# mozack/vdjer

Hardware: AMD Instinct MI355X
Metric: M paired-reads/sec (k-mer build + contig score), IgH 50bp PE (higher is better)
Workload: dtype u8/u64 (2-bit packed bases, integer counts)

## Files before the change

### vdjer_amd/csrc/vdjx_kmer.hip

```cpp
#include "vdjx_common.h"
#include "vdjx_scan.h"
#include "vdjx_part.h"

#include <algorithm>
#include <numeric>
#include <type_traits>
#include <string.h>
#include <stdlib.h>

#define HIST_THREADS 512
#define HIST_BLOCKS 512u
#define LOCAL_SLOTS 2048u
#define K3_SUB_TUPLES g_sub_tuples
__device__ u32 g_sub_tuples = 262144u;
#define NONE32 0xFFFFFFFFu
#define INST_MASK 0x7FFFFFFFu

struct RecView {
	u64 bhi, blo, nm, lq;
};

__device__ inline RecView load_rec(const u64* __restrict__ bases, const u64* __restrict__ nmask,
                                   const u64* __restrict__ lowq, size_t r) {
	RecView v;
// ... 1124 lines not shown
	if (r0 == NONE32) return;
	if ((need & NEED_SEQ) && r != r0 && lane == 0) {
		const u64* a = (const u64*) me;
		const u64* b = (const u64*) (replies + (size_t) r0 * REPLY_BYTES);
		u64 d = 0;
#pragma unroll
		for (int w = 2; w < 10; w++) d |= a[w] ^ b[w];
		if (d) p_fl[pid] = 1;
	}
	if ((need & NEED_Q) && (int) lane < k) {
		const uint8_t* first = me + REPLY_Q0 + (r == r0 ? 2 * REPLY_KQ : REPLY_KQ);
		atomicAdd(&p_S[(size_t) pid * 64 + lane], (u32) me[REPLY_Q0 + lane] + (u32) first[lane]);
		if (np) {
			const uint8_t* first_r = me + REPLY_RQ0 + (r == p_r0[np + pid] ? 2 * REPLY_KQ : REPLY_KQ);
			atomicAdd(&p_S[((size_t) np + pid) * 64 + lane], (u32) me[REPLY_RQ0 + lane] + (u32) first_r[lane]);
		}
	}
}

template <bool SYM>
__global__ void k_resolve_keep(PendOut po, u32 np, const u32* __restrict__ p_fl, const u32* __restrict__ p_S, int k, u32 mf, u32 mqq, u32 tlow,
                               SurvOutG so) {
	const u32 p = blockIdx.x * blockDim.x + threadIdx.x;
	const bool in = p < np;
	const u32 need = in ? po.need[p] : 0u;
	bool keep = in && ((need & NEED_SEQ) ? p_fl[p] != 0 : true);
	const u32 cg = in ? po.cg[p] : 0u;
	const u32 cgc = cg > CNT_CAP ? CNT_CAP : cg;
	keep = keep && cgc >= mf;
	bool keep_r = keep;
	if (keep && cg < tlow) {
		for (int j = 0; j < k; j++) if (p_S[(size_t) p * 64 + j] < mqq) { keep = false; break; }
		if (SYM) for (int j = 0; j < k; j++) if (p_S[((size_t) np + p) * 64 + j] < mqq) { keep_r = false; break; }
	}
	if (!SYM) {
		const u32 pos = vdjx_wave_inc(so.n, keep);
		if (keep && pos < so.cap) {
			so.lo[pos] = po.lo[p]; so.hi[pos] = po.hi[p];
			so.gcnt[pos] = cgc; so.gfirst[pos] = po.mg[p];
		}
		return;
	}
	const bool any = keep || keep_r;
	const u32 pos = vdjx_wave_inc(so.n, any, 2u);
	if (any && pos + 1 < so.cap) {
		so.lo[pos] = po.lo[p]; so.hi[pos] = po.hi[p];
		so.gcnt[pos] = cgc | (keep ? 0u : GC_SHADOW); so.gfirst[pos] = po.mg[p];
		u64 rh, rlo;
		vdjx_kmer_rc(po.hi[p], po.lo[p], k, rh, rlo);
		so.lo[pos + 1] = rlo; so.hi[pos + 1] = rh;
		so.gcnt[pos + 1] = cgc | (keep_r ? 0u : GC_SHADOW); so.gfirst[pos + 1] = po.mgr[p];
	}
}

__global__ void k_first_to_scan(u64* __restrict__ a, size_t na, u64* __restrict__ b, size_t nb, const u32* __restrict__ scan, int ob) {
	const size_t i = (size_t) blockIdx.x * blockDim.x + threadIdx.x;
	if (i >= na + nb) return;
	u64* p = i < na ? a + i : b + (i - na);
	const u64 v = *p;
	if (v != NONE64) *p = ((u64) scan[v >> ob] << ob) | (v & ((1ull << ob) - 1ull));
}

__global__ void k_node_flags(const u64* __restrict__ s_lo, const u64* __restrict__ s_hi, u32 n, int k,
                             const u32* __restrict__ vbits, const u32* __restrict__ jbits,
                             uint8_t* __restrict__ has_v, uint8_t* __restrict__ has_j) {
	u32 i = blockIdx.x * blockDim.x + threadIdx.x;
	if (i >= n) return;
	if (k <= 16) { has_v[i] = 1; has_j[i] = 1; return; }
	u128 key = ((u128) s_hi[i] << 64) | s_lo[i];
	u32 code = (u32) (key >> (2 * (k - 16)));
	has_v[i] = code ? (vbits[code >> 5] >> (code & 31)) & 1u : 0;
	has_j[i] = code ? (jbits[code >> 5] >> (code & 31)) & 1u : 0;
}


#define IT_INST_BITS 35
#define IT_INST_MASK ((1ull << IT_INST_BITS) - 1ull)
#define IT_SURV_SHIFT 38
#define IT_HOLE 0xFFFFFFFFFFFFFFFFull
#define WALK_THREADS 256

#define SLOT_HI_BITS 36
#define SLOT_HI_MASK ((1ull << SLOT_HI_BITS) - 1ull)
struct SurvTable { const ulonglong2* slots; u32 mask; const ulonglong2* skey; const u32* bloom; u32 bloom_mask; };

struct ItemFmt {
	u32 pmask;
	u32 len_shift;
	u32 maxlen;
	u32 mul, inv;
	u32 bmask;
	u32 ns;
};
__device__ inline u32 it_surv(const ItemFmt& f, u64 x) { return (u32) (x >> IT_SURV_SHIFT) & f.pmask; }
__device__ inline u32 it_len(const ItemFmt& f, u64 x) { return f.maxlen > 1 ? (u32) (x >> f.len_shift) + 1u : 1u; }
__device__ inline u32 it_scat(const ItemFmt& f, u32 p) { return ((((p >> 4) * f.mul) & f.bmask) << 4) | (p & 15u); }

__global__ void k_surv_table2(const u64* __restrict__ s_lo, const u64* __restrict__ s_hi, u32 n, ulonglong2* __restrict__ slots, u32 mask,
                              ulonglong2* __restrict__ skey, u32* __restrict__ bloom, u32 bloom_mask) {
	const u32 i = blockIdx.x * blockDim.x + threadIdx.x;
	if (i >= n) return;
	const u64 lo = s_lo[i], hi = s_hi[i];
	skey[i] = make_ulonglong2(lo, hi);
	const u64 h = vdjx_mix(lo, hi);
	{
		const u32 bit = (u32) (h >> 40) & bloom_mask;
		atomicOr(&bloom[bit >> 5], 1u << (bit & 31));
	}
	u32 slot = (u32) (h >> 20) & mask;
	const unsigned long long entry = hi | ((unsigned long long) (i + 1) << SLOT_HI_BITS);
	while (atomicCAS((unsigned long long*) &slots[slot].y, 0ull, entry) != 0ull) slot = (slot + 1) & mask;
	slots[slot].x = lo;
}

__device__ inline int surv_lookup2f(const SurvTable& t, u64 lo, u64 hi);

__device__ inline int surv_lookup2(const SurvTable& t, u64 lo, u64 hi) {
	u32 slot = (u32) (vdjx_mix(lo, hi) >> 20) & t.mask;
	for (;;) {
		const ulonglong2 v = t.slots[slot];
		if (!v.y) return -1;
		if (v.x == lo && (v.y & SLOT_HI_MASK) == hi) return (int) (v.y >> SLOT_HI_BITS) - 1;
		slot = (slot + 1) & t.mask;
	}
}

__device__ inline int surv_lookup2f(const SurvTable& t, u64 lo, u64 hi) {
	const u64 h = vdjx_mix(lo, hi);
	const u32 bit = (u32) (h >> 40) & t.bloom_mask;
	if (!((t.bloom[bit >> 5] >> (bit & 31)) & 1u)) return -1;
	return surv_lookup2(t, lo, hi);
}

__global__ void k_succ_links2(SurvTable t, u32 n, int k, const u32* __restrict__ gcnt, u32* __restrict__ succ, unsigned long long* __restrict__ pred,
                              u32* __restrict__ bestsucc) {
	const u32 u = blockIdx.x * blockDim.x + threadIdx.x;
	if (u >= n) return;
	const ulonglong2 kk = t.skey[u];
	const u128 base = (((u128) kk.y << 64) | kk.x) << 2;
	const u128 km = k < 64 ? (((u128) 1) << (2 * k)) - 1 : ~(u128) 0;
	const int sh = 2 * (k - 1);
	const u32 fb = (u32) (sh < 64 ? kk.x >> sh : kk.y >> (sh - 64)) & 3u;
	const unsigned long long mine = ((unsigned long long) (gcnt[u] & GC_MASK) << 32) | ((unsigned long long) (fb ^ 1u) << 30) | (unsigned long long) u;
	u32 best = NONE32, best_g = 0;
	for (u32 b = 0; b < 4; b++) {
		const u128 key = (base | (u128) b) & km;
		const int s = surv_lookup2(t, (u64) key, (u64) (key >> 64));
		succ[u * 4 + b] = s >= 0 ? (u32) s : NONE32;
		if (s >= 0 && (u32) s != u) {
			const u32 g = gcnt[s] & GC_MASK;
			if (best == NONE32 || g >= best_g) { best = (u32) s; best_g = g; }
			atomicMax(&pred[s], mine);
		}
	}
	bestsucc[u] = best;
}

#define CHAIN_JUMPS 31
__global__ void k_chain_init(const unsigned long long* __restrict__ pred, const u32* __restrict__ bestsucc, u32 n, u64* __restrict__ pd) {
	const u32 v = blockIdx.x * blockDim.x + threadIdx.x;
	if (v >= n) return;
	const unsigned long long x = pred[v];
	const u32 u = (u32) x & 0x3FFFFFFFu;
	pd[v] = x != 0ull && bestsucc[u] == v ? ((u64) u << 32) | 1ull : ((u64) NONE32 << 32);
}

__global__ void k_partner(SurvTable t, u32 n, int k, u32* __restrict__ partner) {
	const u32 p = blockIdx.x * blockDim.x + threadIdx.x;
	if (p >= n) return;
	const ulonglong2 kk = t.skey[p];
	u64 rh, rlo;
	vdjx_kmer_rc(kk.y, kk.x, k, rh, rlo);
	const int q = surv_lookup2(t, rlo, rh);
	partner[p] = q >= 0 ? (u32) q : NONE32;
}
__global__ void k_partner_check(const u32* __restrict__ partner, const u64* __restrict__ linw, u32 n, u32* __restrict__ bad) {
	const u32 p = blockIdx.x * blockDim.x + threadIdx.x;
	if (p >= n) return;
	bool wrong = partner[p] == NONE32;
	const bool linked = (linw[p >> 4] >> (15u - (p & 15u))) & 1ull;
	if (!wrong && linked && (p + 1 >= n || partner[p + 1] != partner[p] - 1u)) wrong = true;
	const u64 m = __ballot(wrong);
	if (m && __lane_id() == 0) atomicAdd(bad, (u32) __popcll(m));
}

__global__ void k_chain_jump(u64* __restrict__ pd, u32 n, const u32* __restrict__ open_prev, u32* __restrict__ open_now) {
	if (open_prev && *open_prev == 0) return;
	const u32 v = blockIdx.x * blockDim.x + threadIdx.x;
	bool open = false;
	if (v < n) {
		u64 x = __atomic_load_n(&pd[v], __ATOMIC_RELAXED);
		for (int it = 0; it < CHAIN_JUMPS; it++) {
			const u32 p = (u32) (x >> 32);
			if (p == NONE32) break;
			const u64 y = __atomic_load_n(&pd[p], __ATOMIC_RELAXED);
			const u32 pp = (u32) (y >> 32);
			if (pp == NONE32) break;
			x = ((u64) pp << 32) | (u64) ((u32) x + (u32) y);
			__atomic_store_n(&pd[v], x, __ATOMIC_RELAXED);
			open = true;
		}
	}
	if (__ballot(open) && __lane_id() == 0) atomicAdd(open_now, 1u);
}

__device__ inline void chain_of(const u64* pd, u32 v, u32& head, u32& dist) {
	const u64 x = pd[v];
	const u32 p = (u32) (x >> 32);
	head = v; dist = 0;
	if (p == NONE32) return;
	if ((u32) (pd[p] >> 32) != NONE32) return;
	head = p; dist = (u32) x;
}
__global__ void k_chain_len(const u64* __restrict__ pd, u32 n, u32* __restrict__ len) {
	const u32 v = blockIdx.x * blockDim.x + threadIdx.x;
	if (v >= n) return;
	u32 h, d;
	chain_of(pd, v, h, d);
	atomicAdd(&len[h], 1u);
}

__global__ void k_chain_place(const u64* __restrict__ pd, const u32* __restrict__ off, u32 n, u32* __restrict__ newidx) {
	const u32 v = blockIdx.x * blockDim.x + threadIdx.x;
	if (v >= n) return;
	u32 h, d;
	chain_of(pd, v, h, d);
	newidx[v] = off[h] + d;
}
__global__ void k_chain_permute(const u32* __restrict__ newidx, u32 n, const u64* __restrict__ lo, const u64* __restrict__ hi, const u32* __restrict__ gcnt,
                                const u64* __restrict__ gfirst, const u32* __restrict__ succ, u64* __restrict__ lo2, u64* __restrict__ hi2,
                                u32* __restrict__ gcnt2, u64* __restrict__ gfirst2, ulonglong2* __restrict__ skey2, u32* __restrict__ succ2) {
	const u32 v = blockIdx.x * blockDim.x + threadIdx.x;
	if (v >= n) return;
	const u32 q = newidx[v];
	const u64 l = lo[v], h = hi[v];
	lo2[q] = l; hi2[q] = h; gcnt2[q] = gcnt[v]; gfirst2[q] = gfirst[v];
	skey2[q] = make_ulonglong2(l, h);
	const uint4 s = *(const uint4*) &succ[(size_t) v * 4];
	uint4 r;
	r.x = s.x == NONE32 ? NONE32 : newidx[s.x];
	r.y = s.y == NONE32 ? NONE32 : newidx[s.y];
	r.z = s.z == NONE32 ? NONE32 : newidx[s.z];
	r.w = s.w == NONE32 ? NONE32 : newidx[s.w];
	*(uint4*) &succ2[(size_t) q * 4] = r;
}
__global__ void k_table_remap(ulonglong2* __restrict__ slots, u32 n_slots, const u32* __restrict__ newidx) {
	const u32 i = blockIdx.x * blockDim.x + threadIdx.x;
	if (i >= n_slots) return;
	const u64 y = slots[i].y;
	if (!y) return;
	slots[i].y = (y & SLOT_HI_MASK) | ((u64) (newidx[(u32) (y >> SLOT_HI_BITS) - 1] + 1u) << SLOT_HI_BITS);
}

__global__ void k_chain_words(const u32* __restrict__ succ, const ulonglong2* __restrict__ skey, u32 n, int k, u64* __restrict__ linw, u32* __restrict__ fbw,
                              const u32* __restrict__ partner) {
	const u32 p = blockIdx.x * blockDim.x + threadIdx.x;
	const u32 j = p & 15u;
	u64 w = 0;
	u32 fb = 0;
	if (p < n) {
		const uint4 s = *(const uint4*) &succ[(size_t) p * 4];
		const u32 sv[4] = {s.x, s.y, s.z, s.w};
		const bool mirrored = !partner || (p + 1 < n && partner[p] != NONE32 && partner[p + 1] == partner[p] - 1u);
		for (u32 b = 0; b < 4; b++) if (sv[b] != NONE32) {
			if (sv[b] == p + 1 && mirrored) w |= (1ull << (15u - j)) | ((u64) b << (32u + 2u * (15u - j)));
			else w |= 1ull << (31u - j);
		}
		const ulonglong2 kk = skey[p];
		const int sh = 2 * (k - 1);
		fb = (u32) (sh < 64 ? kk.x >> sh : kk.y >> (sh - 64)) & 3u;
	}
	u32 fw = fb << (2 * j);
	for (int d = 1; d < 16; d <<= 1) {
		w |= ((u64) (u32) __shfl_xor((int) (w >> 32), d) << 32) | (u32) __shfl_xor((int) (u32) w, d);
		fw |= (u32) __shfl_xor((int) fw, d);
	}
	if (j == 0 && p < n) { linw[p >> 4] = w; fbw[p >> 4] = fw; }
}

struct WalkRecS {
	u64 bhi, blo; int rl;
	__device__ inline void kmer_u(int k, int o, u64& hi, u64& lo) const { vdjx_kmer_at(bhi, blo, rl, k, o, hi, lo); }
	__device__ inline void kmer_l(int k, int o, u64& hi, u64& lo) const { vdjx_kmer_at_lane(bhi, blo, rl, k, o, hi, lo); }
	__device__ inline u32 bases16(int bi) const {
		const int sh = 2 * (rl - 16 - bi);
		const u32 rw_dn = vdjx_bits_at_lane(bhi, blo, (u32) (sh > 0 ? sh : 0));
		const u32 up = (u32) (sh < 0 ? -sh : 0);
		return (rw_dn << (up & 31u)) & (0u - (u32) (up < 32u));
	}
	__device__ inline u32 base(int i) const { return vdjx_base_at_lane(bhi, blo, rl, i); }
};
struct WalkRecL {
	const u64* row;
	__device__ inline void kmer_u(int k, int o, u64& hi, u64& lo) const { vdjx_kmer_at_words(row, k, o, hi, lo); }
	__device__ inline void kmer_l(int k, int o, u64& hi, u64& lo) const { vdjx_kmer_at_words(row, k, o, hi, lo); }
	__device__ inline u32 bases16(int bi) const { return vdjx_bases16_words(row, bi); }
	__device__ inline u32 base(int i) const { return vdjx_base_words(row, i); }
};
__device__ inline bool wm_test(u64 m, int i) { return (m >> i) & 1ull; }
__device__ inline bool wm_test(const vdjx_mask3& m, int i) { return m.test(i); }
__device__ inline void wm_set(u64& m, int i) { m |= 1ull << i; }
__device__ inline void wm_set(vdjx_mask3& m, int i) { m.set(i); }
__device__ inline int wm_next(u64 m, int from, int none) { const u64 x = from < 64 ? m & (~0ull << from) : 0ull; return x ? __builtin_ctzll(x) : none; }
__device__ inline int wm_next(const vdjx_mask3& m, int from, int none) { return m.next(from, none); }
__device__ inline u32 wm_slice32(u64 m, int from) { return from < 64 ? (u32) (m >> from) : 0u; }
__device__ inline u32 wm_slice32(const vdjx_mask3& m, int from) { return (u32) m.slice(from); }

template <bool LONG, bool SYM = false>
__global__ __launch_bounds__(WALK_THREADS) void k_walk_items(const u64* __restrict__ bases, const u64* __restrict__ nmask, size_t R, int rl, int ob_bits, int k,
                                                             SurvTable t, const u32* __restrict__ succ, const u64* __restrict__ linw, ItemFmt f,
                                                             u32 range_shift, u32 n_ranges,
                                                             u64* __restrict__ raw, u64 raw_cap, u32 blk_items,
                                                             unsigned long long* __restrict__ g_cursor,
                                                             u32* __restrict__ range_cnt, u32* __restrict__ g_err, u32 dbg_in,
                                                             const u32* __restrict__ partner) {
	static_assert(!(LONG && SYM), "SYM is the short-read form");
#ifdef VDJX_ABLATE
	const u32 dbg = dbg_in;
#else
	(void) dbg_in;
	constexpr u32 dbg = 0u;
#endif
	extern __shared__ u32 hist[];
	typedef typename std::conditional<LONG, vdjx_mask3, u64>::type MaskT;
	typedef typename std::conditional<LONG, WalkRecL, WalkRecS>::type RecT;
	for (u32 i = threadIdx.x; i < n_ranges; i += WALK_THREADS) hist[i] = 0;
	__syncthreads();
	u64* myrow = (u64*) (hist + ((n_ranges + 1u) & ~1u)) + threadIdx.x * GL_ROW_LONG;
	const int P = rl - k + 1;
	const size_t per = ((R + gridDim.x - 1) / gridDim.x + WALK_THREADS - 1) / WALK_THREADS * WALK_THREADS;
	const size_t r0 = (size_t) blockIdx.x * per;
	const size_t r1 = r0 + per < R ? r0 + per : R;
	const int lane = __lane_id();
	u64 blk = 0;
	u32 fill = blk_items;
#ifdef WALK_STATS
	u32 st_rows = 0, st_rounds = 0, st_filter = 0, st_lookup = 0, st_items = 0, st_chain = 0;
#define WST(x) x
#else
#define WST(x)
#endif
	bool have_blk = false, dead = false;
	__shared__ u64 dq[WALK_THREADS / 64][128];
	__shared__ ulonglong2 dq_b[LONG ? 1 : WALK_THREADS / 64][LONG ? 1 : 128];
	__shared__ u64 dq_v[LONG ? 1 : WALK_THREADS / 64][LONG ? 1 : 128];
	const u32 wq = threadIdx.x >> 6;
	u32 qn = 0;
	auto walk_row = [&](auto fresh_tag, const size_t r, const bool live, const int o_from, const ulonglong2 qb, const u64 qv) {
		constexpr bool FRESH = decltype(fresh_tag)::value;
		RecT v;
		MaskT V{};
// ... 261 lines not shown
				const int leader = __ffsll((long long) act) - 1;
				const u32 lslot = (u32) __builtin_amdgcn_readlane((int) slot, leader);
				const bool same = shaped && slot == lslot;
				const u64 m = __ballot(same);
				if (__popcll(m) >= 8) {
					const u64 v64 = inst + 15u - a;
					const u32 hi_min = vdjx_wave_min(same ? (u32) (v64 >> 32) : 0xFFFFFFFFu);
					const u32 lo_min = vdjx_wave_min(same && (u32) (v64 >> 32) == hi_min ? (u32) v64 : 0xFFFFFFFFu);
					if (__lane_id() == leader) {
						const u32 n = (u32) __popcll(m);
						atomicAdd(&c[cb + e], n);
						if (a) atomicAdd(&c[cb + a - 1u], 0u - n);
						rc_min(&mv[lslot], (IT) (((u64) hi_min << 32) | lo_min));
					}
					mine = shaped && !same;
				}
			}
			if (live && (mine || !shaped)) {
				atomicAdd(&c[cb + e], 1u);
				if (a) atomicAdd(&c[cb + a - 1u], 0xFFFFFFFFu);
			}
			if (mine) rc_min(&mv[slot], val);
			if (live && !shaped) {
				const u32 k = 31u - (u32) __builtin_clz(len), w = 1u << k;
				rc_min(&mv[mb + rc_win(k, a)], val);
				if (len != w) rc_min(&mv[mb + rc_win(k, e + 1u - w)], val);
			}
			if (live && ((x >> 37) & 1ull)) {
				IT* ep = &ef[sl * 4 + (u32) ((x >> 35) & 3ull)];
				if (vdjx_peek(ep) > (IT) inst) rc_min(ep, (IT) inst);
			}
		}
	}
	__syncthreads();
	const u64 add = rec_base << ob;
	u32 my_cnt = 0;
	for (u32 i = threadIdx.x; i < SB; i += RC_THREADS) {
		const u32 sb = (s0 + i) >> 4;
		const u32 blk = (sb * f.inv) & f.bmask;
		const u32 x = i & 15u, p = (blk << 4) | x;
		if (sb > f.bmask || blk >= nb || p >= ns) continue;
		const u32 cbase = (i >> 4) * RC_CS, mbase = (i >> 4) * RC_MS;
		u32 cc = 0;
		IT mm = NONE;
		IT me = NONE;
		for (u32 e = x; e < 16; e++) { cc += c[cbase + e]; const IT t = mv[mbase + e]; mm = t < mm ? t : mm; if (x) me = t < me ? t : me; }
		for (u32 a = 1; a <= x; a++) { const IT t = mv[mbase + 15 + a]; mm = t < mm ? t : mm; if (a < x) me = t < me ? t : me; }
#pragma unroll
		for (u32 k = 0; k < 4; k++) {
			const u32 w = 1u << k;
			const u32 lo = x >= w ? x - w + 1u : 1u, hi = x < 15u - w ? x : 15u - w;
			for (u32 s = lo ? lo : 1u; s <= hi; s++) { const IT t = mv[mbase + rc_win(k, s)]; mm = t < mm ? t : mm; if (s < x) me = t < me ? t : me; }
		}
		my_cnt += cc;
		ucnt[p] = cc;
		ufirst[p] = mm == NONE ? NONE64 : (u64) mm - 15u + x + add;
		IT e4[4] = {ef[i * 4], ef[i * 4 + 1], ef[i * 4 + 2], ef[i * 4 + 3]};
		if (x && me != NONE) {
			const u32 pa = (fbl[i >> 4] >> (2 * (x - 1))) & 3u;
			const IT t = (IT) (me - 15u + x);
			if (t < e4[pa]) e4[pa] = t;
		}
		for (u32 q = 0; q < 4; q++) in_first[(size_t) p * 4 + q] = e4[q] == NONE ? NONE64 : (u64) e4[q] + add;
	}
	if (my_cnt) atomicAdd(&tot, (unsigned long long) my_cnt);
	__syncthreads();
	if (threadIdx.x == 0 && tot) atomicAdd(n_inst, tot);
}

__global__ void k_count_unseen(const u64* __restrict__ ufirst, u32 n, u32* __restrict__ out) {
	const u32 i = blockIdx.x * blockDim.x + threadIdx.x;
	const bool un = i < n && ufirst[i] == NONE64;
	const u64 m = __ballot(un);
	if (m && __lane_id() == 0) atomicAdd(out, (u32) __popcll(m));
}

__global__ void k_edges_from_in(SurvTable t, u32 n, int k, const u64* __restrict__ in_first, u32* __restrict__ in_from,
                                u64* __restrict__ edge_first, u32* __restrict__ edge_to) {
	const u32 e = blockIdx.x * blockDim.x + threadIdx.x;
	if (e >= n * 4u) return;
	const u64 fs = in_first[e];
	if (fs == NONE64) { in_from[e] = NONE32; return; }
	const u32 v = e >> 2, a = e & 3u;
	const ulonglong2 kk = t.skey[v];
	const u128 kv = ((u128) kk.y << 64) | kk.x;
	const u128 ku = (kv >> 2) | ((u128) a << (2 * (k - 1)));
	const int u = surv_lookup2(t, (u64) ku, (u64) (ku >> 64));
	in_from[e] = u >= 0 ? (u32) u : NONE32;
	if (u >= 0) {
		const u32 oe = (u32) u * 4u + ((u32) kk.x & 3u);
		edge_first[oe] = fs;
		edge_to[oe] = v;
	}
}

struct SurvRec { u64 lo, hi; u32 gcnt, pad; u64 gfirst; };

__global__ void k_surv_pack(const u64* __restrict__ lo, const u64* __restrict__ hi, const u32* __restrict__ gcnt,
                            const u64* __restrict__ gfirst, u32 n, SurvRec* __restrict__ out) {
	u32 i = blockIdx.x * blockDim.x + threadIdx.x;
	if (i >= n) return;
	SurvRec r{lo[i], hi[i], gcnt[i], 0u, gfirst[i]};
	out[i] = r;
}

__global__ void k_surv_unpack(const SurvRec* __restrict__ in, u32 n, u64* __restrict__ lo, u64* __restrict__ hi, u32* __restrict__ gcnt,
                              u64* __restrict__ gfirst, u32* __restrict__ n_real) {
	u32 i = blockIdx.x * blockDim.x + threadIdx.x;
	const bool in_range = i < n;
	SurvRec r{0, 0, GC_SHADOW, 0, 0};
	if (in_range) {
		r = in[i];
		lo[i] = r.lo; hi[i] = r.hi; gcnt[i] = r.gcnt; gfirst[i] = r.gfirst;
	}
	(void) vdjx_wave_inc(n_real, in_range && !(r.gcnt & GC_SHADOW));
}

struct NodeOut {
	u64* first_inst; u32* gcnt; u32* freq; uint8_t* hv; uint8_t* hj; u64* klo; u64* khi; char* kmers;
	uint8_t* to_deg; u32* to_ids; uint8_t* from_deg; u32* from_ids;
};

__global__ void k_rank_keys(const u64* __restrict__ ufirst, const u32* __restrict__ gcnt, u32 n, u64* __restrict__ key, u32* __restrict__ idx) {
	const u32 i = blockIdx.x * blockDim.x + threadIdx.x;
	if (i < n) { key[i] = (gcnt[i] & GC_SHADOW) ? NONE64 : ufirst[i]; idx[i] = i; }
}
__global__ void k_rank_scatter(const u64* __restrict__ key, const u32* __restrict__ idx, u32 n, u32* __restrict__ rank) {
	const u32 j = blockIdx.x * blockDim.x + threadIdx.x;
	if (j >= n) return;
	const u32 i = idx[j];
	rank[i] = key[j] == NONE64 ? i : j;
}

__global__ __launch_bounds__(256) void k_root_count(const uint8_t* __restrict__ from_deg, u32 n, u32* __restrict__ block_cnt) {
	__shared__ u32 cnt;
	if (threadIdx.x == 0) cnt = 0;
	__syncthreads();
	const u32 i = blockIdx.x * 256 + threadIdx.x;
	const bool r = i < n && from_deg[i] == 0;
	const u64 b = __ballot(r);
	if ((threadIdx.x & 63) == 0 && b) atomicAdd(&cnt, (u32) __popcll(b));
	__syncthreads();
	if (threadIdx.x == 0) block_cnt[blockIdx.x] = cnt;
}

__global__ __launch_bounds__(256) void k_root_list(const uint8_t* __restrict__ from_deg, u32 n, const u32* __restrict__ block_start,
                                                   u32* __restrict__ roots) {
	__shared__ u32 wave_cnt[4];
	const u32 i = blockIdx.x * 256 + threadIdx.x;
	const bool r = i < n && from_deg[i] == 0;
	const u64 b = __ballot(r);
	const u32 w = threadIdx.x >> 6, lane = threadIdx.x & 63;
	if (lane == 0) wave_cnt[w] = (u32) __popcll(b);
	__syncthreads();
	u32 base = block_start[blockIdx.x];
	for (u32 j = 0; j < w; j++) base += wave_cnt[j];
	if (r) roots[base + (u32) __popcll(b & ((1ull << lane) - 1))] = i;
}

__device__ inline void sort4_desc64(u64 (&f)[4], u32 (&id)[4]) {
#define CSW(a, b) { const bool sw = kk[a] < kk[b]; if (sw) { u64 t = kk[a]; kk[a] = kk[b]; kk[b] = t; u32 u = id[a]; id[a] = id[b]; id[b] = u; } }
	u64 kk[4];
	for (int i = 0; i < 4; i++) kk[i] = f[i] == NONE64 ? 0ull : f[i] + 1;
	CSW(0, 1) CSW(2, 3) CSW(0, 2) CSW(1, 3) CSW(1, 2)
	for (int i = 0; i < 4; i++) f[i] = kk[i] ? kk[i] - 1 : NONE64;
#undef CSW
}
// ... 327 lines not shown

template <typename TUP, typename A>
int stage_gated_reduce(vdjx_ctx* c, A& db, GTuples<TUP>& t, const PoolView& pv, u64 rec_base, int k, int mf, int mq, SurvivorsG* sv, bool sym = false) {
	hipStream_t st = c->stream;
	int rc = set_sub_tuples(c);
	if (rc) return rc;
	if (mq >= 255) mq = 254;
	const u32 mqq = (u32) (mq < 0 ? 0 : (mq > 214 ? 214 : mq));
	const u32 tlow = 1 + (mqq + 19) / 20;
	const u32 cmin = (u32) std::max(mf, 2);
	const u32 mfu = (u32) std::max(mf, 0);
	const u32 cap = (sym ? t.Nsurv : t.Nsurv / 2) + 16;
	u32 *g_err, *n_surv;
	u64* g_distinct;
	HIP_TRY(db.alloc(&sv->lo, cap)); HIP_TRY(db.alloc(&sv->hi, cap)); HIP_TRY(db.alloc(&sv->gcnt, cap)); HIP_TRY(db.alloc(&sv->gfirst, cap));
	HIP_TRY(db.alloc(&g_distinct, 64 * 16 + 3));
	g_err = (u32*) (g_distinct + 64 * 16);
	n_surv = g_err + 1;
	u32* n_real = g_err + 2;
	HIP_TRY(hipMemsetAsync(g_distinct, 0, (64 * 16 + 3) * 8, st));
	if (t.over) hipLaunchKernelGGL(k_cut_totals, dim3((t.NB + 1023) / 1024), dim3(1024), 0, st, t.bucket_start, t.bucket_end, t.NB, (const u32*) t.over, g_err + 3,
	                               (unsigned long long*) (g_distinct + 64 * 16 + 2));
	SurvOutG so{sv->lo, sv->hi, sv->gcnt, sv->gfirst, n_surv, cap, n_real};
	static const u32 rd_dbg = (u32) vdjx_env_num("VDJX_RD_DBG", 0, 0, 9);
	if (t.N) {
		vdjx_prof_scope ps(c, "k_gated_reduce");
		u32* order;
		if ((rc = bucket_order(c, db, t, &order))) return rc;
		if (sym) hipLaunchKernelGGL((k_gated_reduce<TUP, true>), dim3(t.NB), dim3(RD_THREADS), 0, st, t.t, t.bucket_start, t.bucket_end, (const u32*) t.over, pv.bases, pv.nmask, pv.quals, pv.rl, pv.ob, k, rec_base,
		                            mfu, cmin, mqq, tlow, so, g_distinct, g_err, rd_dbg, (const u32*) order);
		else hipLaunchKernelGGL(k_gated_reduce<TUP>, dim3(t.NB), dim3(RD_THREADS), 0, st, t.t, t.bucket_start, t.bucket_end, (const u32*) t.over, pv.bases, pv.nmask, pv.quals, pv.rl, pv.ob, k, rec_base,
		                        mfu, cmin, mqq, tlow, so, g_distinct, g_err, rd_dbg, (const u32*) order);
	}
	u64* spread = (u64*) c->h_pin;
	u32* tail = (u32*) (spread + 64 * 16);
	static_assert((64 * 16 + 3) * 8 == VDJX_HPIN_SYNC_BYTES, "h_pin layout (vdjx_common.h)");
	HIP_TRY(hipMemcpyAsync(spread, g_distinct, VDJX_HPIN_SYNC_BYTES, hipMemcpyDeviceToHost, st));
	HIP_TRY(hipStreamSynchronize(st));
	HIP_TRY(hipGetLastError());
	const u32 ns = tail[1], err = tail[0];
	if (t.over) {
		if (tail[3] || ns > cap) return VDJX_ECUT;
		t.N = (u32) spread[64 * 16 + 2];
		c->stats["gated_instances"] = sym ? 2ull * t.N : t.N;
	}
	if (err) { vdjx_set_error("k_gated_reduce: %u buckets could not be split to fit LDS", err); return VDJX_EHIP; }
	if (ns > cap) { vdjx_set_error("survivor capacity logic failed (%u > %u)", ns, cap); return VDJX_EHIP; }
	sv->ndist = 0;
	for (int i = 0; i < 64; i++) sv->ndist += spread[i * 16];
	sv->n = ns;
	sv->n_real = sym ? tail[2] : ns;
	c->stats["kmer_build_shadows"] = ns - sv->n_real;
	return VDJX_OK;
}

struct RecountOut { u32* ucnt; u64* ufirst; u64* in_first; u32* in_from; u64* edge_first; u32* edge_to; };
struct RecountStatus { const u32* g_err = nullptr; const u32* n_items = nullptr; const unsigned long long* n_inst = nullptr; u32 ns = 0; };
#define VDJX_ESYMWALK (-1000)
static int recount_status_check(vdjx_ctx* c, const u32* hp, u32 ns) {
	if (hp[6] || hp[7]) { vdjx_set_error("the mirrored walk found %u + %u places where the chains are not mirror images", hp[6], hp[7]); return VDJX_ESYMWALK; }
	if (hp[0]) { vdjx_set_error("k_walk_items: item buffer too small (%u waves stopped)", hp[0]); return VDJX_EHIP; }
	if (hp[1]) { vdjx_set_error("internal error: %u of %u surviving k-mers were not met again in the records (VDJX_SYNC_DEBUG=1 names them)", hp[1], ns); return VDJX_EHIP; }
	c->stats["recount_items"] = hp[2];
	c->stats["recount_instances"] = *(const unsigned long long*) (hp + 4);
	return VDJX_OK;
}

template <typename A>
int stage_recount(vdjx_ctx* c, A& db, const vdjx_pool* pool, u64 rec_base, int k, SurvivorsG& sv, const RecountOut& ro,
                  bool derive_edges, SurvTable* table_out = nullptr, RecountStatus* defer = nullptr, bool sym_walk = false) {
	hipStream_t st = c->stream;
	const size_t R = pool->n_records;
	const int P = pool->rl - k + 1;
	const u32 ns = sv.n;
	if (ns >= (1u << 26)) { vdjx_set_error("more than 2^26 surviving k-mers: not supported by the recount items"); return VDJX_ELIMIT; }
	if (R >= (1ull << 29)) { vdjx_set_error("more than 2^29 records on one GPU: not supported by the recount items"); return VDJX_ELIMIT; }
	if ((u64) R * (u64) P >= (1ull << 32)) { vdjx_set_error("records*offsets = %llu >= 2^32 on one GPU: shard the pool over more GPUs", (unsigned long long) ((u64) R * (u64) P)); return VDJX_ELIMIT; }
	u32 tmask = 1023;
	while ((size_t) tmask + 1 < (size_t) ns * 2) tmask = tmask * 2 + 1;
	unsigned long long* pred;
	ulonglong2* table;
	u32 *succ0, *succ, *bloom, *clen, *coff, *newidx, *jump_open, *fbw, *gcnt2, *bestsucc, *partner = nullptr;
	u64 *pd, *lo2, *hi2, *gfirst2, *linw;
	ulonglong2 *skey0, *skey;
	u32 bloom_bits = 1u << 16;
	while (bloom_bits < (1u << 30) && (size_t) bloom_bits < (size_t) ns * 16) bloom_bits <<= 1;
	const u32 nb16 = (ns + 15u) >> 4;
	const u32 n_jump = (ceil_log2_u64((u64) ns + 1) + 4) / 5 + 1;
	{
		auto up = [](size_t b) { return (b + 255) & ~(size_t) 255; };
		const size_t b_bloom = up(bloom_bits / 8), b_table = up(((size_t) tmask + 1) * 16), b_pred = up((size_t) ns * 8), b_clen = up((size_t) ns * 4),
		             b_jump = up((size_t) (n_jump + 1) * 4), b_linw = up(((size_t) nb16 + 1) * 8);
		uint8_t* z;
		const size_t zb = b_bloom + b_table + b_pred + b_clen + b_jump + b_linw;
		HIP_TRY(db.alloc(&z, zb));
		HIP_TRY(hipMemsetAsync(z, 0, zb, st));
		table = (ulonglong2*) z; z += b_table;
		bloom = (u32*) z; z += b_bloom;
		pred = (unsigned long long*) z; z += b_pred;
		clen = (u32*) z; z += b_clen;
		jump_open = (u32*) z; z += b_jump;
		linw = (u64*) z;
	}
	HIP_TRY(db.alloc(&skey0, ns)); HIP_TRY(db.alloc(&skey, ns));
	HIP_TRY(db.alloc(&succ0, (size_t) ns * 4)); HIP_TRY(db.alloc(&succ, (size_t) ns * 4));
	HIP_TRY(db.alloc(&pd, ns)); HIP_TRY(db.alloc(&coff, (size_t) ns + 1)); HIP_TRY(db.alloc(&newidx, ns));
	HIP_TRY(db.alloc(&lo2, ns)); HIP_TRY(db.alloc(&hi2, ns)); HIP_TRY(db.alloc(&gcnt2, ns)); HIP_TRY(db.alloc(&gfirst2, ns));
	HIP_TRY(db.alloc(&fbw, nb16));
	HIP_TRY(db.alloc(&bestsucc, ns));
	if (sym_walk) HIP_TRY(db.alloc(&partner, ns));
	const SurvTable tb0{table, tmask, skey0, bloom, bloom_bits - 1};
	const SurvTable tb{table, tmask, skey, bloom, bloom_bits - 1};
	if (table_out) *table_out = tb;
	const dim3 gs((ns + 255) / 256), bs(256);
	{
		vdjx_prof_scope ps(c, "k_surv_table");
		hipLaunchKernelGGL(k_surv_table2, gs, bs, 0, st, sv.lo, sv.hi, ns, table, tmask, skey0, bloom, bloom_bits - 1);
		hipLaunchKernelGGL(k_succ_links2, gs, bs, 0, st, tb0, ns, k, sv.gcnt, succ0, pred, bestsucc);
	}
	{
		vdjx_prof_scope ps(c, "k_chain_order");
		hipLaunchKernelGGL(k_chain_init, gs, bs, 0, st, pred, bestsucc, ns, pd);
		for (u32 j = 0; j < n_jump; j++) hipLaunchKernelGGL(k_chain_jump, gs, bs, 0, st, pd, ns, j ? jump_open + j - 1 : (const u32*) nullptr, jump_open + j);
		hipLaunchKernelGGL(k_chain_len, gs, bs, 0, st, pd, ns, clen);
		{ const int rc_ = vdjx_scan_wide(db, st, clen, ns, coff); if (rc_) return rc_; }
		hipLaunchKernelGGL(k_chain_place, gs, bs, 0, st, pd, coff, ns, newidx);
		hipLaunchKernelGGL(k_chain_permute, gs, bs, 0, st, newidx, ns, sv.lo, sv.hi, sv.gcnt, sv.gfirst, succ0, lo2, hi2, gcnt2, gfirst2, skey, succ);
		hipLaunchKernelGGL(k_table_remap, dim3(tmask / 256 + 1), bs, 0, st, table, tmask + 1, newidx);
		if (sym_walk) hipLaunchKernelGGL(k_partner, gs, bs, 0, st, tb, ns, k, partner);
		hipLaunchKernelGGL(k_chain_words, gs, bs, 0, st, succ, skey, ns, k, linw, fbw, (const u32*) partner);
	}
	dbg_sync(c, "k_chain_order");
	if (sync_debug()) {
		std::vector<u32> ni(ns), seen(ns, 0);
		(void) hipMemcpy(ni.data(), newidx, (size_t) ns * 4, hipMemcpyDeviceToHost);
		u32 dup = 0, oob = 0;
		for (u32 i = 0; i < ns; i++) { if (ni[i] >= ns) oob++; else if (seen[ni[i]]++) dup++; }
		std::vector<u64> pdh(ns);
		std::vector<unsigned long long> prh(ns);
		(void) hipMemcpy(pdh.data(), pd, (size_t) ns * 8, hipMemcpyDeviceToHost);
		(void) hipMemcpy(prh.data(), pred, (size_t) ns * 8, hipMemcpyDeviceToHost);
		u32 unresolved = 0;
		for (u32 i = 0; i < ns; i++) { const u32 p0 = (u32) (pdh[i] >> 32); if (p0 != NONE32 && (u32) (pdh[p0] >> 32) != NONE32) unresolved++; }
		fprintf(stderr, "[vdjx] chain order: %u survivors, %u duplicate new indices, %u out of range, %u unresolved (cycles), %u jump launches\n", ns, dup, oob, unresolved, n_jump);
		for (u32 i = 0, shown = 0; i < ns && shown < 6; i++) if (ni[i] < ns && seen[ni[i]] > 1) {
			fprintf(stderr, "[vdjx]   old %u -> new %u: pd = (%u, %u), pred word %llx\n", i, ni[i], (u32) (pdh[i] >> 32), (u32) pdh[i], prh[i]);
			shown++;
		}
	}
	sv.lo = lo2; sv.hi = hi2; sv.gcnt = gcnt2; sv.gfirst = gfirst2;
	ItemFmt f;
	{
		const u32 sb = ceil_log2_u64(ns);
		static const u32 force_lb = (u32) vdjx_env_num("VDJX_RC_LEN_BITS", 4, 0, 4);
		const u32 lb = std::min(std::min(4u, 26u - sb), force_lb);
		const u32 pb = 26u - lb;
		f.pmask = (1u << pb) - 1u;
		f.len_shift = IT_SURV_SHIFT + pb;
		f.maxlen = 1u << lb;
		const u32 t = ceil_log2_u64(nb16);
		f.bmask = (1u << t) - 1u;
		f.mul = t ? ((0x9E3779B9u >> (32 - t)) | 1u) : 1u;
		u32 x = f.mul;
		for (int i = 0; i < 5; i++) x *= 2u - f.mul * x;
		f.inv = x & f.bmask;
		f.ns = ns;
	}
	const u32 nsp = (f.bmask + 1u) << 4;
	static const bool force_wide = vdjx_env_num("VDJX_RC_WIDE", 0, 0, 1) != 0;
	static const u32 cap_shift = (u32) vdjx_env_num("VDJX_RC_MAX_SHIFT", 12, 8, 12);
	const bool narrow = R < (1ull << (32 - pool->ob)) && !force_wide;
	static const u32 max_ranges = (u32) vdjx_env_num("VDJX_RC_MAX_RANGES", PART_MAXB, 2, PART_MAXB);
	const u32 max_shift = std::max(8u, std::min(narrow ? 11u : 10u, cap_shift));
	u32 range_shift = 8;
	while (range_shift < max_shift && (nsp >> range_shift) > max_ranges) range_shift++;
	const u32 n_ranges = std::max(1u, nsp >> range_shift);
	u32 l2bits = 0;
	while (((n_ranges + (1u << l2bits) - 1) >> l2bits) > max_ranges) l2bits++;
	if (l2bits) l2bits = std::min(10u, std::max(l2bits, (ceil_log2_u64(n_ranges) + 1u) / 2u));
	const u32 n_coarse = (n_ranges + (1u << l2bits) - 1) >> l2bits;
	const u32 n_ranges_p = n_coarse << l2bits;
	constexpr size_t walk_blocks = 7168;
	const size_t Rw = sym_walk ? R / 2 : R;
	u32 nblk = (u32) std::min<size_t>(walk_blocks, (Rw + WALK_THREADS * 8 - 1) / (WALK_THREADS * 8));
	constexpr u32 walk_resident = 1536;
	if (nblk > walk_resident && nblk < walk_blocks) nblk = nblk / walk_resident * walk_resident;
	if (nblk < walk_resident) nblk = (u32) std::min<size_t>(walk_resident, (Rw + WALK_THREADS - 1) / WALK_THREADS);
	if (nblk == 0) nblk = 1;
	const size_t nwaves = (size_t) nblk * (WALK_THREADS / 64);
	const size_t NI = R * (size_t) P;
	u32 blk_items = 4096;
	while (blk_items > 256 && nwaves * blk_items > NI / 2 + 65536) blk_items >>= 1;
	const u64 raw_cap = (u64) NI + (u64) NI / (blk_items / 64) + nwaves * (u64) blk_items + blk_items;
	u64 *raw, *items;
	unsigned long long *g_cursor, *n_inst;
	u32 *range_cnt, *range_start, *g_err, *gcur;
	const vdjx_arena::mark_t tmp_mark = db.mark();
	HIP_TRY(db.alloc(&raw, (size_t) raw_cap));
	HIP_TRY(db.alloc(&g_cursor, 4 + ((size_t) n_ranges_p + 1) / 2));
	n_inst = g_cursor + 1;
	g_err = (u32*) (g_cursor + 2);
	range_cnt = (u32*) (g_cursor + 4);
	HIP_TRY(db.alloc(&range_start, n_ranges_p + 1));
	HIP_TRY(hipMemsetAsync(g_cursor, 0, 32 + (size_t) n_ranges_p * 4, st));
	if (sym_walk) {
		vdjx_prof_scope ps(c, "k_chain_order");
		hipLaunchKernelGGL(k_partner_check, gs, bs, 0, st, partner, linw, ns, g_err + 3);
	}
	const bool lng = pool->W > 2;
	if (lng && R >= (1ull << 27)) { vdjx_set_error("more than 2^27 records of long reads on one GPU: not supported by the recount items"); return VDJX_ELIMIT; }
	const size_t lds_walk = (((size_t) n_ranges_p + 1) & ~(size_t) 1) * 4 + (lng ? (size_t) WALK_THREADS * GL_ROW_LONG * 8 : 0);
	if ((size_t) n_ranges_p * 4 > 64 * 1024) { vdjx_set_error("too many survivor ranges for the walk histogram"); return VDJX_ELIMIT; }
	HIP_TRY(hipFuncSetAttribute((const void*) k_walk_items<false>, hipFuncAttributeMaxDynamicSharedMemorySize, (int) lds_walk));
// ... 965 lines not shown
```

Measured before the change: 969.6.

## Drop skey copies, fuse chain length into last jump, remap table via slot numbers

Removes the interleaved skey arrays and reads keys from the existing lo/hi arrays. The table is remapped from recorded slot numbers inside the permute kernel, replacing a full-table remap pass. The chain-length kernel and its atomics are folded into a final templated jump launch that writes lengths directly. pred zeroing moves into the table-build kernel and shrinks the memset, and successor lookups now go through the bloom filter. Together this cuts launches and memory traffic, at the cost of split key loads and more complex length logic that must stay correct.

```diff
diff --git a/vdjer_amd/csrc/vdjx_kmer.hip b/vdjer_amd/csrc/vdjx_kmer.hip
--- a/vdjer_amd/csrc/vdjx_kmer.hip
+++ b/vdjer_amd/csrc/vdjx_kmer.hip
@@ -1230,7 +1230,8 @@
 
 #define SLOT_HI_BITS 36
 #define SLOT_HI_MASK ((1ull << SLOT_HI_BITS) - 1ull)
-struct SurvTable { const ulonglong2* slots; u32 mask; const ulonglong2* skey; const u32* bloom; u32 bloom_mask; };
+struct SurvTable { const ulonglong2* slots; u32 mask; const u64* klo; const u64* khi; const u32* bloom; u32 bloom_mask; };
+__device__ inline ulonglong2 surv_key(const SurvTable& t, u32 i) { return make_ulonglong2(t.klo[i], t.khi[i]); }
 
 struct ItemFmt {
 	u32 pmask;
@@ -1245,11 +1246,11 @@
 __device__ inline u32 it_scat(const ItemFmt& f, u32 p) { return ((((p >> 4) * f.mul) & f.bmask) << 4) | (p & 15u); }
 
 __global__ void k_surv_table2(const u64* __restrict__ s_lo, const u64* __restrict__ s_hi, u32 n, ulonglong2* __restrict__ slots, u32 mask,
-                              ulonglong2* __restrict__ skey, u32* __restrict__ bloom, u32 bloom_mask) {
+                              u32* __restrict__ bloom, u32 bloom_mask, u32* __restrict__ slotno, unsigned long long* __restrict__ pred) {
 	const u32 i = blockIdx.x * blockDim.x + threadIdx.x;
 	if (i >= n) return;
 	const u64 lo = s_lo[i], hi = s_hi[i];
-	skey[i] = make_ulonglong2(lo, hi);
+	pred[i] = 0ull;
 	const u64 h = vdjx_mix(lo, hi);
 	{
 		const u32 bit = (u32) (h >> 40) & bloom_mask;
@@ -1259,6 +1260,7 @@
 	const unsigned long long entry = hi | ((unsigned long long) (i + 1) << SLOT_HI_BITS);
 	while (atomicCAS((unsigned long long*) &slots[slot].y, 0ull, entry) != 0ull) slot = (slot + 1) & mask;
 	slots[slot].x = lo;
+	slotno[i] = slot;
 }
 
 __device__ inline int surv_lookup2f(const SurvTable& t, u64 lo, u64 hi);
@@ -1284,7 +1286,7 @@
                               u32* __restrict__ bestsucc) {
 	const u32 u = blockIdx.x * blockDim.x + threadIdx.x;
 	if (u >= n) return;
-	const ulonglong2 kk = t.skey[u];
+	const ulonglong2 kk = surv_key(t, u);
 	const u128 base = (((u128) kk.y << 64) | kk.x) << 2;
 	const u128 km = k < 64 ? (((u128) 1) << (2 * k)) - 1 : ~(u128) 0;
 	const int sh = 2 * (k - 1);
@@ -1293,7 +1295,7 @@
 	u32 best = NONE32, best_g = 0;
 	for (u32 b = 0; b < 4; b++) {
 		const u128 key = (base | (u128) b) & km;
-		const int s = surv_lookup2(t, (u64) key, (u64) (key >> 64));
+		const int s = surv_lookup2f(t, (u64) key, (u64) (key >> 64));
 		succ[u * 4 + b] = s >= 0 ? (u32) s : NONE32;
 		if (s >= 0 && (u32) s != u) {
 			const u32 g = gcnt[s] & GC_MASK;
@@ -1316,7 +1318,7 @@
 __global__ void k_partner(SurvTable t, u32 n, int k, u32* __restrict__ partner) {
 	const u32 p = blockIdx.x * blockDim.x + threadIdx.x;
 	if (p >= n) return;
-	const ulonglong2 kk = t.skey[p];
+	const ulonglong2 kk = surv_key(t, p);
 	u64 rh, rlo;
 	vdjx_kmer_rc(kk.y, kk.x, k, rh, rlo);
 	const int q = surv_lookup2(t, rlo, rh);
@@ -1332,13 +1334,16 @@
 	if (m && __lane_id() == 0) atomicAdd(bad, (u32) __popcll(m));
 }
 
-__global__ void k_chain_jump(u64* __restrict__ pd, u32 n, const u32* __restrict__ open_prev, u32* __restrict__ open_now) {
-	if (open_prev && *open_prev == 0) return;
+template <bool LAST>
+__global__ void k_chain_jump(u64* __restrict__ pd, u32 n, const u32* __restrict__ open_prev, u32* __restrict__ open_now,
+                             const unsigned long long* __restrict__ pred, const u32* __restrict__ bestsucc, u32* __restrict__ len) {
+	const bool idle = open_prev && *open_prev == 0;
+	if (!LAST && idle) return;
 	const u32 v = blockIdx.x * blockDim.x + threadIdx.x;
 	bool open = false;
 	if (v < n) {
 		u64 x = __atomic_load_n(&pd[v], __ATOMIC_RELAXED);
-		for (int it = 0; it < CHAIN_JUMPS; it++) {
+		if (!idle) for (int it = 0; it < CHAIN_JUMPS; it++) {
 			const u32 p = (u32) (x >> 32);
 			if (p == NONE32) break;
 			const u64 y = __atomic_load_n(&pd[p], __ATOMIC_RELAXED);
@@ -1348,8 +1353,20 @@
 			__atomic_store_n(&pd[v], x, __ATOMIC_RELAXED);
 			open = true;
 		}
-	}
-	if (__ballot(open) && __lane_id() == 0) atomicAdd(open_now, 1u);
+		if (LAST) {
+			const u32 p = (u32) (x >> 32);
+			const bool head = p == NONE32;
+			if (!head && (u32) (__atomic_load_n(&pd[p], __ATOMIC_RELAXED) >> 32) != NONE32) len[v] = 1u;
+			else {
+				const u32 s = bestsucc[v];
+				const unsigned long long ps = s != NONE32 ? pred[s] : 0ull;
+				const bool linked = ps != 0ull && ((u32) ps & 0x3FFFFFFFu) == v;
+				if (!head) len[v] = 0u;
+				if (!linked) len[head ? v : p] = (head ? 0u : (u32) x) + 1u;
+			}
+		}
+	}
+	if (!idle && __ballot(open) && __lane_id() == 0) atomicAdd(open_now, 1u);
 }
 
 __device__ inline void chain_of(const u64* pd, u32 v, u32& head, u32& dist) {
@@ -1360,13 +1377,6 @@
 	if ((u32) (pd[p] >> 32) != NONE32) return;
 	head = p; dist = (u32) x;
 }
-__global__ void k_chain_len(const u64* __restrict__ pd, u32 n, u32* __restrict__ len) {
-	const u32 v = blockIdx.x * blockDim.x + threadIdx.x;
-	if (v >= n) return;
-	u32 h, d;
-	chain_of(pd, v, h, d);
-	atomicAdd(&len[h], 1u);
-}
 
 __global__ void k_chain_place(const u64* __restrict__ pd, const u32* __restrict__ off, u32 n, u32* __restrict__ newidx) {
 	const u32 v = blockIdx.x * blockDim.x + threadIdx.x;
@@ -1377,13 +1387,14 @@
 }
 __global__ void k_chain_permute(const u32* __restrict__ newidx, u32 n, const u64* __restrict__ lo, const u64* __restrict__ hi, const u32* __restrict__ gcnt,
                                 const u64* __restrict__ gfirst, const u32* __restrict__ succ, u64* __restrict__ lo2, u64* __restrict__ hi2,
-                                u32* __restrict__ gcnt2, u64* __restrict__ gfirst2, ulonglong2* __restrict__ skey2, u32* __restrict__ succ2) {
+                                u32* __restrict__ gcnt2, u64* __restrict__ gfirst2, u32* __restrict__ succ2,
+                                const u32* __restrict__ slotno, ulonglong2* __restrict__ slots) {
 	const u32 v = blockIdx.x * blockDim.x + threadIdx.x;
 	if (v >= n) return;
 	const u32 q = newidx[v];
 	const u64 l = lo[v], h = hi[v];
 	lo2[q] = l; hi2[q] = h; gcnt2[q] = gcnt[v]; gfirst2[q] = gfirst[v];
-	skey2[q] = make_ulonglong2(l, h);
+	slots[slotno[v]].y = h | ((u64) (q + 1u) << SLOT_HI_BITS);
 	const uint4 s = *(const uint4*) &succ[(size_t) v * 4];
 	uint4 r;
 	r.x = s.x == NONE32 ? NONE32 : newidx[s.x];
@@ -1392,15 +1403,8 @@
 	r.w = s.w == NONE32 ? NONE32 : newidx[s.w];
 	*(uint4*) &succ2[(size_t) q * 4] = r;
 }
-__global__ void k_table_remap(ulonglong2* __restrict__ slots, u32 n_slots, const u32* __restrict__ newidx) {
-	const u32 i = blockIdx.x * blockDim.x + threadIdx.x;
-	if (i >= n_slots) return;
-	const u64 y = slots[i].y;
-	if (!y) return;
-	slots[i].y = (y & SLOT_HI_MASK) | ((u64) (newidx[(u32) (y >> SLOT_HI_BITS) - 1] + 1u) << SLOT_HI_BITS);
-}
-
-__global__ void k_chain_words(const u32* __restrict__ succ, const ulonglong2* __restrict__ skey, u32 n, int k, u64* __restrict__ linw, u32* __restrict__ fbw,
+
+__global__ void k_chain_words(const u32* __restrict__ succ, const u64* __restrict__ klo, const u64* __restrict__ khi, u32 n, int k, u64* __restrict__ linw, u32* __restrict__ fbw,
                               const u32* __restrict__ partner) {
 	const u32 p = blockIdx.x * blockDim.x + threadIdx.x;
 	const u32 j = p & 15u;
@@ -1414,7 +1418,7 @@
 			if (sv[b] == p + 1 && mirrored) w |= (1ull << (15u - j)) | ((u64) b << (32u + 2u * (15u - j)));
 			else w |= 1ull << (31u - j);
 		}
-		const ulonglong2 kk = skey[p];
+		const ulonglong2 kk = make_ulonglong2(klo[p], khi[p]);
 		const int sh = 2 * (k - 1);
 		fb = (u32) (sh < 64 ? kk.x >> sh : kk.y >> (sh - 64)) & 3u;
 	}
@@ -1842,7 +1846,7 @@
 	const u64 fs = in_first[e];
 	if (fs == NONE64) { in_from[e] = NONE32; return; }
 	const u32 v = e >> 2, a = e & 3u;
-	const ulonglong2 kk = t.skey[v];
+	const ulonglong2 kk = surv_key(t, v);
 	const u128 kv = ((u128) kk.y << 64) | kk.x;
 	const u128 ku = (kv >> 2) | ((u128) a << (2 * (k - 1)));
 	const int u = surv_lookup2(t, (u64) ku, (u64) (ku >> 64));
@@ -2336,53 +2340,54 @@
 	ulonglong2* table;
 	u32 *succ0, *succ, *bloom, *clen, *coff, *newidx, *jump_open, *fbw, *gcnt2, *bestsucc, *partner = nullptr;
 	u64 *pd, *lo2, *hi2, *gfirst2, *linw;
-	ulonglong2 *skey0, *skey;
 	u32 bloom_bits = 1u << 16;
 	while (bloom_bits < (1u << 30) && (size_t) bloom_bits < (size_t) ns * 16) bloom_bits <<= 1;
 	const u32 nb16 = (ns + 15u) >> 4;
 	const u32 n_jump = (ceil_log2_u64((u64) ns + 1) + 4) / 5 + 1;
 	{
 		auto up = [](size_t b) { return (b + 255) & ~(size_t) 255; };
-		const size_t b_bloom = up(bloom_bits / 8), b_table = up(((size_t) tmask + 1) * 16), b_pred = up((size_t) ns * 8), b_clen = up((size_t) ns * 4),
+		const size_t b_bloom = up(bloom_bits / 8), b_table = up(((size_t) tmask + 1) * 16),
 		             b_jump = up((size_t) (n_jump + 1) * 4), b_linw = up(((size_t) nb16 + 1) * 8);
 		uint8_t* z;
-		const size_t zb = b_bloom + b_table + b_pred + b_clen + b_jump + b_linw;
+		const size_t zb = b_bloom + b_table + b_jump + b_linw;
 		HIP_TRY(db.alloc(&z, zb));
 		HIP_TRY(hipMemsetAsync(z, 0, zb, st));
 		table = (ulonglong2*) z; z += b_table;
 		bloom = (u32*) z; z += b_bloom;
-		pred = (unsigned long long*) z; z += b_pred;
-		clen = (u32*) z; z += b_clen;
 		jump_open = (u32*) z; z += b_jump;
 		linw = (u64*) z;
 	}
-	HIP_TRY(db.alloc(&skey0, ns)); HIP_TRY(db.alloc(&skey, ns));
+	u32* slotno;
+	HIP_TRY(db.alloc(&pred, ns)); HIP_TRY(db.alloc(&clen, ns)); HIP_TRY(db.alloc(&slotno, ns));
 	HIP_TRY(db.alloc(&succ0, (size_t) ns * 4)); HIP_TRY(db.alloc(&succ, (size_t) ns * 4));
 	HIP_TRY(db.alloc(&pd, ns)); HIP_TRY(db.alloc(&coff, (size_t) ns + 1)); HIP_TRY(db.alloc(&newidx, ns));
 	HIP_TRY(db.alloc(&lo2, ns)); HIP_TRY(db.alloc(&hi2, ns)); HIP_TRY(db.alloc(&gcnt2, ns)); HIP_TRY(db.alloc(&gfirst2, ns));
 	HIP_TRY(db.alloc(&fbw, nb16));
 	HIP_TRY(db.alloc(&bestsucc, ns));
 	if (sym_walk) HIP_TRY(db.alloc(&partner, ns));
-	const SurvTable tb0{table, tmask, skey0, bloom, bloom_bits - 1};
-	const SurvTable tb{table, tmask, skey, bloom, bloom_bits - 1};
+	const SurvTable tb0{table, tmask, sv.lo, sv.hi, bloom, bloom_bits - 1};
+	const SurvTable tb{table, tmask, lo2, hi2, bloom, bloom_bits - 1};
 	if (table_out) *table_out = tb;
 	const dim3 gs((ns + 255) / 256), bs(256);
 	{
 		vdjx_prof_scope ps(c, "k_surv_table");
-		hipLaunchKernelGGL(k_surv_table2, gs, bs, 0, st, sv.lo, sv.hi, ns, table, tmask, skey0, bloom, bloom_bits - 1);
+		hipLaunchKernelGGL(k_surv_table2, gs, bs, 0, st, sv.lo, sv.hi, ns, table, tmask, bloom, bloom_bits - 1, slotno, pred);
 		hipLaunchKernelGGL(k_succ_links2, gs, bs, 0, st, tb0, ns, k, sv.gcnt, succ0, pred, bestsucc);
 	}
 	{
 		vdjx_prof_scope ps(c, "k_chain_order");
 		hipLaunchKernelGGL(k_chain_init, gs, bs, 0, st, pred, bestsucc, ns, pd);
-		for (u32 j = 0; j < n_jump; j++) hipLaunchKernelGGL(k_chain_jump, gs, bs, 0, st, pd, ns, j ? jump_open + j - 1 : (const u32*) nullptr, jump_open + j);
-		hipLaunchKernelGGL(k_chain_len, gs, bs, 0, st, pd, ns, clen);
+		for (u32 j = 0; j + 1 < n_jump; j++)
+			hipLaunchKernelGGL(k_chain_jump<false>, gs, bs, 0, st, pd, ns, j ? jump_open + j - 1 : (const u32*) nullptr, jump_open + j, (const unsigned long long*) pred,
+			                   (const u32*) bestsucc, clen);
+		hipLaunchKernelGGL(k_chain_jump<true>, gs, bs, 0, st, pd, ns, n_jump > 1 ? jump_open + n_jump - 2 : (const u32*) nullptr, jump_open + n_jump - 1,
+		                   (const unsigned long long*) pred, (const u32*) bestsucc, clen);
 		{ const int rc_ = vdjx_scan_wide(db, st, clen, ns, coff); if (rc_) return rc_; }
 		hipLaunchKernelGGL(k_chain_place, gs, bs, 0, st, pd, coff, ns, newidx);
-		hipLaunchKernelGGL(k_chain_permute, gs, bs, 0, st, newidx, ns, sv.lo, sv.hi, sv.gcnt, sv.gfirst, succ0, lo2, hi2, gcnt2, gfirst2, skey, succ);
-		hipLaunchKernelGGL(k_table_remap, dim3(tmask / 256 + 1), bs, 0, st, table, tmask + 1, newidx);
+		hipLaunchKernelGGL(k_chain_permute, gs, bs, 0, st, newidx, ns, sv.lo, sv.hi, sv.gcnt, sv.gfirst, succ0, lo2, hi2, gcnt2, gfirst2, succ,
+		                   (const u32*) slotno, table);
 		if (sym_walk) hipLaunchKernelGGL(k_partner, gs, bs, 0, st, tb, ns, k, partner);
-		hipLaunchKernelGGL(k_chain_words, gs, bs, 0, st, succ, skey, ns, k, linw, fbw, (const u32*) partner);
+		hipLaunchKernelGGL(k_chain_words, gs, bs, 0, st, succ, (const u64*) lo2, (const u64*) hi2, ns, k, linw, fbw, (const u32*) partner);
 	}
 	dbg_sync(c, "k_chain_order");
 	if (sync_debug()) {
```

Result: faster. 980.8 (median of 6 runs) (+1.2%).
